# retinal-information-processing-lab/gaussian_processes

Measured on AMD Instinct MI355X. Metric: GP fits/sec (kernel+chol+solve+grad loglik) at N=8192 d=256, higher is better.
Workload: dtype f64; 1 GPU; N=8192 d=256 single cell f64, one M-step closure evaluation with 6 gradients (BASELINE configs[2], headline); N=8192, d=256, parallelism=independent units over 1 GPU(s), one process per GPU, no data-path collective

## Files before the change

gaussian_processes_amd/csrc/context.h:

```cpp
#pragma once
#include "kernels.h"
#include <vector>

struct gpfit_ctx {
  int device = 0;
  int np_cap = 0, dp_cap = 0, dfull_cap = 0;
  hipStream_t aux = nullptr;
  hipEvent_t ev_fork = nullptr, ev_join = nullptr;

  double *Kbuf = nullptr, *Cos = nullptr, *Lbuf = nullptr, *Libuf = nullptr, *Vbuf = nullptr, *LVbuf = nullptr,
         *LiVbuf = nullptr, *Tbuf = nullptr, *Zbuf = nullptr, *Wbuf = nullptr, *Abuf = nullptr, *Tmp = nullptr,
         *TmpV = nullptr;
  double *Xt = nullptr, *Xm = nullptr, *XCt = nullptr, *Cmat = nullptr, *Ybuf = nullptr, *Mpart = nullptr,
         *Mmat = nullptr, *Xt2 = nullptr, *XCt2 = nullptr, *XDt = nullptr, *XDt2 = nullptr, *dCpad = nullptr;
  double *Kvec = nullptr, *q = nullptr, *lam_m = nullptr, *lam_var = nullptr, *fvec = nullptr, *wl = nullptr,
         *yv = nullptr, *bv = nullptr, *tvec = nullptr , *mpad = nullptr, *rpad = nullptr,
         *q2 = nullptr, *dq1 = nullptr, *dq2 = nullptr, *hvec = nullptr;
  double *upart = nullptr, *vpart = nullptr, *sumA_part = nullptr, *frob_part = nullptr, *trmv_part = nullptr;
  double* rect_part = nullptr;
  void* sk_ws[2] = {nullptr, nullptr};
  hipStream_t side = nullptr;
  std::vector<hipEvent_t> side_ev;
  int side_ev_next = 0;
  double* scal = nullptr;
  double* scal_host = nullptr;
  int* pix = nullptr;
  int* pix_host = nullptr;
  int* info = nullptr;
  int* info_host = nullptr;
  std::vector<void*> allocs;
  int split_k_M = 32;

  int profile = 0;
  struct ProfRec { hipEvent_t a, b; double flops; int kind; };
  std::vector<ProfRec> prof;
  std::vector<hipEvent_t> ev_pool;
  double prof_out[16] = {0};
  hipEvent_t phase_ev[8] = {nullptr, nullptr, nullptr, nullptr, nullptr, nullptr, nullptr, nullptr};
  bool phase_valid = false;
  double last_enqueue_ms = 0.0;
  struct Pending { bool active = false; hipStream_t stream = nullptr; double A = 0, lambda0 = 0, sigma0 = 0;
                   int n = 0, np = 0, d = 0, want_grad = 0, elem_bytes = 8; hipEvent_t done = nullptr;
                   bool use_done = false; } pend;

  int cur_n = 0, cur_np = 0, cur_d = 0, cur_dp = 0;
  bool lv_valid = false;
  bool lv32_valid = false;
  int lv_n = 0;
  int lv_bytes = 0;
};

namespace gpfit {

struct DeviceGuard {
  int prev = -1;
  bool switched = false;
  explicit DeviceGuard(int device) {
    if (hipGetDevice(&prev) == hipSuccess && prev != device) switched = (hipSetDevice(device) == hipSuccess);
  }
  ~DeviceGuard() {
    if (switched) (void)hipSetDevice(prev);
  }
};
#define GP_CTX_ENTER(c, name)                                                                        \
  if ((c)->pend.active) {                                                                            \
    gpfit::set_error(name ": an asynchronous evaluation is pending on this context (collect it with " \
                          "gpfit_fit_eval_finish first)");                                           \
    return -3;                                                                                       \
  }                                                                                                  \
  gpfit::DeviceGuard _device_guard((c)->device)

void prof_begin(gpfit_ctx* c);
void prof_end(gpfit_ctx* c);
struct ProfScope {
  hipStream_t s; double flops; int kind; hipEvent_t a = nullptr;
  ProfScope(hipStream_t s, double flops, int kind);
  ~ProfScope();
};
template <typename R> double gemm_flops(const GemmArgsT<R>& g, int tile);

template <typename R>
struct CholBatchT {
  int nb = 0;
  R* A[GEMM_MAXB];
  R* L[GEMM_MAXB];
  R* Li[GEMM_MAXB];
  R* Tmp[GEMM_MAXB];
  int* info[GEMM_MAXB];
  int64_t ld = 0;
  void* sk_ws = nullptr;
  gpfit_ctx* ctx = nullptr;
  int side_min = 0;
};
template <typename R>
int potrf_lockstep(const CholBatchT<R>& B, int r0, int n, uint32_t need, hipStream_t s, uint32_t halves = 0);

}
```

gaussian_processes_amd/csrc/fit.hip:

```cpp
#include "context.h"
#include "gemm_core.h"
#include "gpfit_mi355x.h"

#include <algorithm>
#include <chrono>
#include <cmath>
#include <cstdlib>
#include <cstring>
#include <limits>

namespace gpfit {

static thread_local gpfit_ctx* g_prof = nullptr;
static thread_local void* g_main_sk_ws = nullptr;

static const int* walks() {
  static int w[7] = {3, 2, 1, 9, 9, 2, 2};
  static bool init = false;
  if (!init) {
    init = true;
    if (const char* e = getenv("GPFIT_WALKS")) {
      int v[7];
      if (sscanf(e, "%d,%d,%d,%d,%d,%d,%d", &v[0], &v[1], &v[2], &v[3], &v[4], &v[5], &v[6]) == 7)
        for (int i = 0; i < 7; ++i) w[i] = v[i];
// ... 147 lines not shown
                     int* sumsq_entries = nullptr) {
  if (epi_done) *epi_done = false;
  if (sumsq_entries) *sumsq_entries = 0;
  if (cnt <= 0) return 0;
  if (cnt > GEMM_MAXB) {
    set_error("gemm_list: more problems than a pointer batch holds");
    return -3;
  }
  GemmArgsT<R> g = gemm_args<R>(a_kmajor, b_kmajor, M, N, K, alpha, Ap[0], lda, Bp[0], ldb, beta, Cp[0], ldc, out_lower,
                                a_tri, b_tri, reverse, sk_ws);
  static const bool no_batch = getenv("GPFIT_NO_BATCH") != nullptr;
  if (cnt == 1 || gemm_pick_tile(g) == TILE || no_batch) {
    auto problem = [&](int i, bool fused) {
      g.A = Ap[i]; g.B = Bp[i]; g.C = Cp[i];
      g.epi = fused ? epi : 0; g.aux = (fused && auxp) ? auxp[i] : nullptr; g.sumsq = (fused && sumsqp) ? sumsqp[i] : nullptr;
    };
    GemmRoute routes[GEMM_MAXB];
    bool fused = epi != 0;
    for (int i = 0; i < cnt && fused; ++i) {
      problem(i, true);
      routes[i] = gemm_route(g);
      fused = routes[i].epi != 0;
    }
    for (int i = 0; i < cnt; ++i) {
      problem(i, fused);
      GP_TRY(fused ? run_gemm(s, g, routes[i]) : run_gemm(s, g));
    }
    if (epi_done) *epi_done = fused;
    if (fused && sumsq_entries) *sumsq_entries = routes[0].sumsq_entries;
    return 0;
  }
  g.nptr = cnt;
  g.batch = cnt;
  for (int i = 0; i < cnt; ++i) {
    g.Ap[i] = Ap[i]; g.Bp[i] = Bp[i]; g.Cp[i] = Cp[i];
    g.auxp[i] = auxp ? auxp[i] : nullptr; g.sumsqp[i] = sumsqp ? sumsqp[i] : nullptr;
  }
  g.epi = epi;
  GemmRoute r = gemm_route(g);
  if (epi && r.epi == 0) {
    g.epi = 0;
    r = gemm_route(g);
  }
  if (epi_done) *epi_done = g.epi != 0;
  if (sumsq_entries) *sumsq_entries = r.sumsq_entries;
  return run_gemm(s, g, r);
}

template <typename R>
static int bgemm(const CholBatchT<R>& B, hipStream_t s, uint32_t mask, int a_kmajor, int b_kmajor, int M, int N, int K,
                 double alpha, R* const* Ab, int64_t offA, R* const* Bb, int64_t offB, double beta, R* const* Cb,
                 int64_t offC, int out_lower, int a_tri, int b_tri, int reverse, void* sk_ws) {
  const R* Ap[GEMM_MAXB];
  const R* Bp[GEMM_MAXB];
  R* Cp[GEMM_MAXB];
  int cnt = 0;
  for (int b = 0; b < B.nb; ++b)
    if (mask & (1u << b)) {
      Ap[cnt] = Ab[b] + offA; Bp[cnt] = Bb[b] + offB; Cp[cnt] = Cb[b] + offC;
      ++cnt;
    }
  return gemm_list<R>(s, cnt, Ap, Bp, Cp, a_kmajor, b_kmajor, M, N, K, alpha, B.ld, B.ld, beta, B.ld, out_lower, a_tri,
                      b_tri, reverse, sk_ws);
}

template <typename R>
static GemmArgsT<R> batch_args(const CholBatchT<R>& B, uint32_t mask, int a_kmajor, int b_kmajor, int M, int N, int K, double alpha,
                               R* const* Ab, int64_t offA, R* const* Bb, int64_t offB, double beta, R* const* Cb, int64_t offC,
                               int out_lower, int a_tri, int b_tri, int reverse) {
  GemmArgsT<R> g = gemm_args<R>(a_kmajor, b_kmajor, M, N, K, alpha, (const R*)nullptr, B.ld, (const R*)nullptr, B.ld, beta,
                                (R*)nullptr, B.ld, out_lower, a_tri, b_tri, reverse, B.sk_ws);
  int cnt = 0;
  for (int b = 0; b < B.nb; ++b)
    if (mask & (1u << b)) {
      g.Ap[cnt] = Ab[b] + offA; g.Bp[cnt] = Bb[b] + offB; g.Cp[cnt] = Cb[b] + offC;
      ++cnt;
    }
  g.nptr = cnt;
  g.batch = cnt;
  if (cnt > 0) { g.A = g.Ap[0]; g.B = g.Bp[0]; g.C = g.Cp[0]; }
  return g;
}

template <typename R>
int potrf_lockstep(const CholBatchT<R>& B, int r0, int n, uint32_t need, hipStream_t s, uint32_t halves) {
  const int64_t ld = B.ld;
  const uint32_t all = (B.nb >= 32) ? 0xffffffffu : ((1u << B.nb) - 1u);
  auto off = [&](int r, int c) { return (int64_t)r * ld + c; };
  if (n == TILE) {
    ProfScope ps(s, 0.0, 1);
    LeafBatchT<R> bt{};
    bt.n = B.nb;
    for (int b = 0; b < B.nb; ++b) {
      bt.A[b] = B.A[b] + off(r0, r0); bt.L[b] = B.L[b] + off(r0, r0); bt.Li[b] = B.Li[b] + off(r0, r0);
      bt.info[b] = B.info[b];
    }
    bt.lda = bt.ldl = bt.ldi = ld;
    bt.info_base = r0;
    return launch_chol_leaf_batch(bt, s);
  }
  const int k = n / TILE;
  const int n1 = ((k + 1) / 2) * TILE, n2 = n - n1;
  const int r1 = r0 + n1;
  GP_TRY(potrf_lockstep<R>(B, r0, n1, all, s));
  GP_TRY(bgemm<R>(B, s, all, 0, 0, n2, n1, n1, 1.0, B.A, off(r1, r0), B.Li, off(r0, r0), 0.0, B.L, off(r1, r0), 0, 0, 2,
                  walks()[0], B.sk_ws));
  hipEvent_t joined = nullptr;
  if (need && B.ctx && B.side_min > 0 && n >= B.side_min && B.ctx->side) {
    gpfit_ctx* c = B.ctx;
    auto next_event = [&]() {
      if (c->side_ev_next == (int)c->side_ev.size()) {
        hipEvent_t e = nullptr;
        (void)hipEventCreateWithFlags(&e, hipEventDisableTiming);
        c->side_ev.push_back(e);
      }
      return c->side_ev[c->side_ev_next++];
    };
    hipEvent_t fork = next_event();
    joined = next_event();
    GP_HIP(hipEventRecord(fork, s));
    GP_HIP(hipStreamWaitEvent(c->side, fork, 0));
    GP_TRY(bgemm<R>(B, c->side, need, 0, 1, n2, n1, n1, 1.0, B.L, off(r1, r0), B.Li, off(r0, r0), 0.0, B.Tmp, off(r1, r0), 0, 0,
                    1, walks()[1], c->sk_ws[1]));
    GP_HIP(hipEventRecord(joined, c->side));
  }
  bool merged = false;
  if (need && !joined) {
    static const bool no_batch = getenv("GPFIT_NO_BATCH") != nullptr;
    const GemmArgsT<R> g2 = batch_args<R>(B, all, 0, 0, n2, n2, n1, -1.0, B.L, off(r1, r0), B.L, off(r1, r0), 1.0, B.A, off(r1, r1),
                                          1, 0, 0, 0);
    const GemmArgsT<R> g3 = batch_args<R>(B, need, 0, 1, n2, n1, n1, 1.0, B.L, off(r1, r0), B.Li, off(r0, r0), 0.0, B.Tmp,
                                          off(r1, r0), 0, 0, 1, walks()[1]);
    const GemmRoute pr = no_batch ? GemmRoute{} : gemm_pair_shape(g2, g3);
    if (!no_batch && pr.rc == 0) {
      if (gemm_log_eval() >= 0 && g_eval_count == gemm_log_eval())
        fprintf(stderr, "[gpfit gemm] pair: M %d N %d K %d lower 1 nb %d + M %d N %d K %d btri 1 nb %d tile %d flops %.6e\n", g2.M, g2.N,
                g2.K, g2.nptr, g3.M, g3.N, g3.K, g3.nptr, pr.tile, gemm_flops(g2, pr.tile) + gemm_flops(g3, pr.tile));
      ProfScope ps(s, g_prof ? gemm_flops(g2, pr.tile) + gemm_flops(g3, pr.tile) : 0.0, 3);
      GP_TRY(launch_gemm_pair(g2, g3, pr, s));
      merged = true;
    }
  }
  if (!merged)
    GP_TRY(bgemm<R>(B, s, all, 0, 0, n2, n2, n1, -1.0, B.L, off(r1, r0), B.L, off(r1, r0), 1.0, B.A, off(r1, r1), 1, 0, 0, 0,
                    B.sk_ws));
  GP_TRY(potrf_lockstep<R>(B, r1, n2, need | halves, s));
  if (need) {
    if (joined) GP_HIP(hipStreamWaitEvent(s, joined, 0));
    else if (!merged)
      GP_TRY(bgemm<R>(B, s, need, 0, 1, n2, n1, n1, 1.0, B.L, off(r1, r0), B.Li, off(r0, r0), 0.0, B.Tmp, off(r1, r0), 0, 0,
                      1, walks()[1], B.sk_ws));
    GP_TRY(bgemm<R>(B, s, need, 0, 1, n2, n1, n2, -1.0, B.Li, off(r1, r1), B.Tmp, off(r1, r0), 0.0, B.Li, off(r1, r0), 0, 1, 0,
                    walks()[2], B.sk_ws));
  }
  return 0;
}

template int potrf_lockstep<double>(const CholBatchT<double>&, int, int, uint32_t, hipStream_t, uint32_t);
template int potrf_lockstep<float>(const CholBatchT<float>&, int, int, uint32_t, hipStream_t, uint32_t);

template <typename R>
struct TwoSidedBufs {
  const R* Q; const R* Li; R* W; R* Z; R* H; int64_t ld; int min_split;
  void* sk_ws = nullptr;
};
template <typename R>
static int dual_update_list(hipStream_t s, int cnt, const R* const* Ap, const R* const* Bp, R* const* Hp, R* const* Zp, int M,
                            int N, int K, double alpha, int64_t ld, int b_tri, int walk, void* sk_ws) {
  bool fused = false;
  if (fused_epilogues() & 4) {
    GemmArgsT<R> g = gemm_args<R>(0, 1, M, N, K, alpha, Ap[0], ld, Bp[0], ld, 0.0, Hp[0], ld, 0, 0, b_tri, walk, sk_ws);
    g.epi = 4; g.aux = Zp[0];
    static const bool no_batch = getenv("GPFIT_NO_BATCH") != nullptr;
    if (cnt > 1 && gemm_pick_tile(g) != TILE && !no_batch) { g.nptr = cnt; g.batch = cnt; }
    fused = gemm_route(g).epi != 0;
  }
  if (fused) {
    bool done = false;
    GP_TRY(gemm_list<R>(s, cnt, Ap, Bp, Hp, 0, 1, M, N, K, alpha, ld, ld, 0.0, ld, 0, 0, b_tri, walk, sk_ws, 4, Zp, nullptr, &done));
    if (!done) {
      set_error("two_sided: the dual-update epilogue was announced but not carried");
      return -100;
    }
    return 0;
  }
  for (int i = 0; i < cnt; ++i)
    GP_HIP(hipMemcpy2DAsync(Hp[i], (size_t)ld * sizeof(R), Zp[i], (size_t)ld * sizeof(R), (size_t)N * sizeof(R), (size_t)M,
                            hipMemcpyDeviceToDevice, s));
  GP_TRY(gemm_list<R>(s, cnt, Ap, Bp, Hp, 0, 1, M, N, K, alpha, ld, ld, 1.0, ld, 0, 0, b_tri, walk, sk_ws));
  for (int i = 0; i < cnt; ++i) GP_TRY(launch_axpby_block<R>(Zp[i], ld, Hp[i], ld, M, N, 1.0, 1.0, s));
  return 0;
}

template <typename R>
static int two_sided_list(int cnt, const TwoSidedBufs<R>* b, const int* r0, int n, hipStream_t s) {
  if (cnt <= 0) return 0;
  const int64_t ld = b[0].ld;
  auto at = [&](const R* base, int r, int c) { return const_cast<R*>(base) + (int64_t)r * ld + c; };
  const R* Ap[GEMM_MAXB];
  const R* Bp[GEMM_MAXB];
  R* Cp[GEMM_MAXB];
  const int k = n / TILE;
  if (n < b[0].min_split || k < 2) {
    static const int wbase_walk = getenv("GPFIT_WBASE_WALK") ? atoi(getenv("GPFIT_WBASE_WALK")) : 0;
    for (int i = 0; i < cnt; ++i) { Ap[i] = at(b[i].Q, r0[i], r0[i]); Bp[i] = at(b[i].Li, r0[i], r0[i]); Cp[i] = at(b[i].Z, r0[i], r0[i]); }
    GP_TRY(gemm_list<R>(s, cnt, Ap, Bp, Cp, 1, 1, n, n, n, 1.0, ld, ld, 0.0, ld, 0, 0, 1, walks()[5], b[0].sk_ws));
    for (int i = 0; i < cnt; ++i) { Ap[i] = at(b[i].Li, r0[i], r0[i]); Bp[i] = at(b[i].Z, r0[i], r0[i]); Cp[i] = at(b[i].W, r0[i], r0[i]); }
    GP_TRY(gemm_list<R>(s, cnt, Ap, Bp, Cp, 1, 1, n, n, n, 0.5, ld, ld, 0.0, ld, 1, 2, 0, wbase_walk, b[0].sk_ws));
    return 0;
  }
  const int n1 = ((k + 1) / 2) * TILE, n2 = n - n1;
  auto diagonal_blocks = [&]() -> int {
    TwoSidedBufs<R> bb[GEMM_MAXB];
    int rr[GEMM_MAXB];
    if (n1 == n2 && 2 * cnt <= GEMM_MAXB) {
      for (int i = 0; i < cnt; ++i) {
        bb[2 * i] = b[i]; rr[2 * i] = r0[i];
        bb[2 * i + 1] = b[i]; rr[2 * i + 1] = r0[i] + n1;
      }
      return two_sided_list<R>(2 * cnt, bb, rr, n1, s);
    }
    for (int i = 0; i < cnt; ++i) rr[i] = r0[i] + n1;
    GP_TRY(two_sided_list<R>(cnt, b, r0, n1, s));
    return two_sided_list<R>(cnt, b, rr, n2, s);
  };
  for (int i = 0; i < cnt; ++i) {
    const int r1 = r0[i] + n1;
    Ap[i] = at(b[i].Q, r1, r1); Bp[i] = at(b[i].Li, r1, r0[i]); Cp[i] = at(b[i].Z, r1, r0[i]);
  }
// ... 288 lines not shown
}
static int projected_kl_products(gpfit_ctx* c, hipStream_t s, int nk, int nb) {
  double *Ki = c->Vbuf, *S2 = c->LVbuf, *S3 = c->LiVbuf, *S4 = c->TmpV;
  const int64_t lb = nb;
  GP_TRY(gemm<double>(s, 0, 1, nb, nb, nb, 1.0, Ki, lb, S2, lb, 0.0, S3, lb, 0, 0, 0));
  GP_TRY(launch_proj_trace(S3, lb, nk, c->scal + 5, s));
  return gemm<double>(s, 0, 1, nb, nb, nb, 1.0, S3, lb, Ki, lb, 0.0, S4, lb, 0, 0, 0);
}

static double sigma0_row_metric(const double* sc, double sigma0) { return sigma0 * (2.0 * sc[9] + 2.0 * sc[7]); }
static void grad_rows(const double* sc, double sigma0_row, double* g6) {
  g6[0] = sigma0_row;
  g6[1] = sc[13];
  g6[2] = sc[14];
  g6[3] = sc[11];
  g6[4] = sc[12];
  g6[5] = sc[10];
}
static int assemble_out(gpfit_ctx* c, double A, double lambda0, double sigma0_row, int pad, int d, int want_grad,
                        const char* err_K, const char* err_V, double* out_host) {
  const double* sc = c->scal_host;
  const double loglik = A * sc[0] + lambda0 * sc[1] - sc[2];
  const double trKinvV = sc[5] - (double)pad;
  const double logdetV = sc[40];
  const double KL = -0.5 * logdetV + 0.5 * sc[3] + 0.5 * sc[6] + 0.5 * trKinvV;
  out_host[0] = -(loglik - KL);
  out_host[1] = loglik;
  out_host[2] = KL;
  if (want_grad) grad_rows(sc, sigma0_row, out_host + 3);
  else
    for (int i = 0; i < 6; ++i) out_host[3 + i] = 0.0;
  out_host[9] = sc[3];
  out_host[10] = logdetV;
  out_host[11] = trKinvV;
  out_host[12] = sc[6];
  out_host[13] = (double)d;
  out_host[14] = (double)c->info_host[0];
  out_host[15] = (double)c->info_host[1];
  if (c->info_host[0] != 0) {
    set_error(err_K);
    return c->info_host[0];
  }
  if (c->info_host[1] != 0) {
    set_error(err_V);
    return c->info_host[1];
  }
  return 0;
}

template <typename R>
struct PostJoin {
  const R *Li, *L, *LV, *Cos, *bv, *q, *wl, *Xm, *Cmat;
  R *T, *W, *Z, *H, *A, *Y, *tvec, *Mpart, *Mmat;
};
template <typename R>
static PostJoin<R> post_join_args(gpfit_ctx* c) {
  auto RP = ws_as<R>;
  return PostJoin<R>{RP(c->Libuf), RP(c->Lbuf), RP(c->LVbuf), RP(c->Cos), RP(c->bv), RP(c->q), RP(c->wl), RP(c->Xm), RP(c->Cmat),
                     RP(c->Tbuf), RP(c->Wbuf), RP(c->Zbuf), RP(c->Tmp), RP(c->Abuf), RP(c->Ybuf), RP(c->tvec),
                     RP(c->Mpart), RP(c->Mmat)};
}
static int demote_for_mixed(gpfit_ctx* c, bool reuse_V, int np, int dp, bool blocks, hipStream_t s, PostJoin<float>* pf) {
  auto F = ws_as<float>;
  const int64_t nn = (int64_t)np * np;
  GP_TRY((launch_reduce_slices<double, float>(c->Libuf, nn, 1, F(c->Kbuf), nn, s)));
  if (blocks) {
    const int kt = np / TILE, n1 = ((kt + 1) / 2) * TILE;
    GP_TRY(launch_demote_block(c->Lbuf + (int64_t)n1 * np, np, F(c->Kbuf) + (int64_t)n1 * np, np, np - n1, n1, s));
  }
  if (!(reuse_V && c->lv32_valid)) GP_TRY((launch_reduce_slices<double, float>(c->LVbuf, nn, 1, F(c->Vbuf), nn, s)));
  c->lv32_valid = true;
  GP_TRY((launch_reduce_slices<double, float>(c->Cos, nn, 1, F(c->TmpV), nn, s)));
  GP_TRY((launch_reduce_slices<double, float>(c->bv, np, 1, F(c->q2), np, s)));
  GP_TRY((launch_reduce_slices<double, float>(c->q, np, 1, F(c->dq1), np, s)));
  GP_TRY((launch_reduce_slices<double, float>(c->wl, np, 1, F(c->dq2), np, s)));
  GP_TRY((launch_reduce_slices<double, float>(c->Xm, (int64_t)np * dp, 1, F(c->Xt2), (int64_t)np * dp, s)));
  GP_TRY((launch_reduce_slices<double, float>(c->Cmat, (int64_t)dp * dp, 1, F(c->dCpad), (int64_t)dp * dp, s)));
  *pf = PostJoin<float>{F(c->Kbuf), F(c->Kbuf), F(c->Vbuf), F(c->TmpV), F(c->q2), F(c->dq1), F(c->dq2), F(c->Xt2), F(c->dCpad),
                        F(c->Tbuf), F(c->Wbuf), F(c->Zbuf), F(c->Tmp), F(c->Abuf), F(c->Ybuf), F(c->tvec),
                        F(c->Mpart), F(c->Mmat)};
  return 0;
}

template <typename R>
static int t_in_blocks(int cnt, gpfit_ctx* const* cs, const PostJoin<R>* a, int np, hipStream_t s) {
  const int64_t ld = np;
  const R* Ap[GEMM_MAXB];
  const R* Bp[GEMM_MAXB];
  R* Cp[GEMM_MAXB];
  R* Tp[GEMM_MAXB];
  double* Sp[GEMM_MAXB];
  const int kt = np / TILE, n1 = ((kt + 1) / 2) * TILE, n2 = np - n1;
  int ent = 0;
  auto asks = [&](int M, int Nn, int K, int lower, int a_tri, int b_tri, int walk) {
    GemmArgsT<R> g1 = gemm_args<R>(0, 1, M, Nn, K, 1.0, a[0].Li, ld, a[0].LV, ld, 0.0, a[0].T, ld, lower, a_tri, b_tri, walk, cs[0]->sk_ws[0]);
    g1.epi = 2; g1.sumsq = cs[0]->frob_part;
    return (fused_epilogues() & 2) ? gemm_route(g1).sumsq_entries : 0;
  };
  const bool any_fused = asks(n1, n1, n1, 1, 1, 1, walks()[3]) > 0 || asks(n2, n2, n2, 1, 1, 1, walks()[3]) > 0 ||
                         asks(n2, n1, n2, 0, 1, 0, walks()[2]) > 0;
  auto diag_blocks = [&](int cb, const int* rb, int nblk) -> int {
    const int tb = nblk / TILE;
    int e = asks(nblk, nblk, nblk, 1, 1, 1, walks()[3]);
    const bool ask = e > 0;
    if (!ask) e = tb * (tb + 1) / 2;
    int m = 0;
    for (int i = 0; i < cnt; ++i)
      for (int j = 0; j < cb; ++j, ++m) {
        const int64_t o = (int64_t)rb[j] * ld + rb[j];
        Ap[m] = a[i].Li + o; Bp[m] = a[i].LV + o; Tp[m] = a[i].T + o; Sp[m] = cs[i]->frob_part + ent + j * e;
      }
    bool normed = false;
    GP_TRY(gemm_list<R>(s, m, Ap, Bp, Tp, 0, 1, nblk, nblk, nblk, 1.0, ld, ld, 0.0, ld, 1, 1, 1, walks()[3], cs[0]->sk_ws[0],
                        ask ? 2 : 0, nullptr, Sp, &normed));
    if (normed != ask) {
      set_error("post_join: the tile-norm epilogue of a diagonal block of T was announced but not carried");
      return -100;
    }
    if (!normed && any_fused)
      for (int q = 0; q < m; ++q) GP_TRY(launch_frob_tiles<R>(Tp[q], ld, nblk, nblk, 1, Sp[q], s));
    ent += cb * e;
    return 0;
  };
  const int r_both[2] = {0, n1};
  if (n2 == n1 && 2 * cnt <= GEMM_MAXB) GP_TRY(diag_blocks(2, r_both, n1));
  else {
    GP_TRY(diag_blocks(1, r_both, n1));
    GP_TRY(diag_blocks(1, r_both + 1, n2));
  }
  {
    const int64_t o21 = (int64_t)n1 * ld;
    for (int i = 0; i < cnt; ++i) {
      GP_HIP(hipMemcpy2DAsync(a[i].Z + o21, (size_t)ld * sizeof(R), a[i].LV + o21, (size_t)ld * sizeof(R), (size_t)n1 * sizeof(R),
                              (size_t)n2, hipMemcpyDeviceToDevice, s));
      Ap[i] = a[i].L + o21; Bp[i] = a[i].T; Cp[i] = a[i].Z + o21;
    }
    GP_TRY(gemm_list<R>(s, cnt, Ap, Bp, Cp, 0, 1, n2, n1, n1, -1.0, ld, ld, 1.0, ld, 0, 0, 1, walks()[1], cs[0]->sk_ws[0]));
    int e = asks(n2, n1, n2, 0, 1, 0, walks()[2]);
    const bool ask = e > 0;
    if (!ask) e = (n2 / TILE) * (n1 / TILE);
    for (int i = 0; i < cnt; ++i) {
      Ap[i] = a[i].Li + o21 + n1; Bp[i] = a[i].Z + o21; Tp[i] = a[i].T + o21; Sp[i] = cs[i]->frob_part + ent;
    }
    bool normed = false;
    GP_TRY(gemm_list<R>(s, cnt, Ap, Bp, Tp, 0, 1, n2, n1, n2, 1.0, ld, ld, 0.0, ld, 0, 1, 0, walks()[2], cs[0]->sk_ws[0],
                        ask ? 2 : 0, nullptr, Sp, &normed));
    if (normed != ask) {
      set_error("post_join: the tile-norm epilogue of T21 was announced but not carried");
      return -100;
    }
    if (!normed && any_fused)
      for (int i = 0; i < cnt; ++i) GP_TRY(launch_frob_tiles<R>(Tp[i], ld, n2, n1, 0, Sp[i], s));
    ent += e;
  }
  for (int i = 0; i < cnt; ++i) {
    if (any_fused) GP_TRY(launch_frob_finish(cs[i]->frob_part, ent, cs[i]->scal + 5, s));
    else GP_TRY(launch_frob_lower(a[i].T, ld, np, cs[i]->scal + 5, cs[i]->frob_part, s));
  }
  return 0;
}

template <typename R, typename PhaseFn>
static int post_join_list(int cnt, gpfit_ctx* const* cs, const PostJoin<R>* a, const Theta* th, int n, int np, const int* d,
                          const int* dp, int n_rows, int n_cols, int want_grad, bool blocks, hipStream_t s, PhaseFn&& phase) {
  const int64_t ld = np;
  const R* Ap[GEMM_MAXB];
  const R* Bp[GEMM_MAXB];
  R* Cp[GEMM_MAXB];
  R* Sp2[GEMM_MAXB];
  double* Sp[GEMM_MAXB];
  if (cnt <= 0 || cnt > GEMM_MAXB) return cnt == 0 ? 0 : -3;
  if (!blocks) {
    for (int i = 0; i < cnt; ++i) { Ap[i] = a[i].Li; Bp[i] = a[i].LV; Cp[i] = a[i].T; Sp[i] = cs[i]->frob_part; }
    bool normed = false;
    int norm_entries = 0;
    GP_TRY(gemm_list<R>(s, cnt, Ap, Bp, Cp, 0, 1, np, np, np, 1.0, ld, ld, 0.0, ld, 1, 1, 1, walks()[3], cs[0]->sk_ws[0],
                        (fused_epilogues() & 2) ? 2 : 0, nullptr, Sp, &normed, &norm_entries));
    for (int i = 0; i < cnt; ++i) {
      if (normed) GP_TRY(launch_frob_finish(cs[i]->frob_part, norm_entries, cs[i]->scal + 5, s));
      else GP_TRY(launch_frob_lower(a[i].T, ld, np, cs[i]->scal + 5, cs[i]->frob_part, s));
    }
  } else {
    GP_TRY(t_in_blocks<R>(cnt, cs, a, np, s));
  }
  phase(4, s);
  if (!want_grad) return 0;
  {
    for (int i = 0; i < cnt; ++i) { Ap[i] = a[i].T; Bp[i] = a[i].T; Cp[i] = a[i].W; }
    bool mirrored = false;
    GP_TRY(gemm_list<R>(s, cnt, Ap, Bp, Cp, 0, 0, np, np, np, -1.0, ld, ld, 0.0, ld, 1, 1, 2, walks()[4], cs[0]->sk_ws[0],
                        (fused_epilogues() & 1) ? 1 : 0, nullptr, nullptr, &mirrored));
    for (int i = 0; i < cnt; ++i) {
      GP_TRY(launch_add_diag(a[i].W, ld, np, 1.0, s));
      if (!mirrored) GP_TRY(launch_symmetrize(a[i].W, ld, np, s));
    }
  }
  phase(5, s);
  {
    static const int ts_min = getenv("GPFIT_TS_MIN") ? atoi(getenv("GPFIT_TS_MIN")) : 4096;
    TwoSidedBufs<R> tb[GEMM_MAXB];
    const R* Lf[GEMM_MAXB];
    for (int i = 0; i < cnt; ++i) {
      tb[i] = TwoSidedBufs<R>{a[i].W, a[i].Li, a[i].T, a[i].Z, a[i].H, ld, ts_min > 0 ? ts_min : (1 << 30)};
      tb[i].sk_ws = cs[0]->sk_ws[0];
      Lf[i] = a[i].L;
    }
    if (blocks) GP_TRY(two_sided_top<R>(cnt, tb, Lf, np, s));
    else {
      int r0[GEMM_MAXB];
      for (int i = 0; i < cnt; ++i) r0[i] = 0;
      GP_TRY(two_sided_list<R>(cnt, tb, r0, np, s));
    }
  }
  phase(6, s);
  for (int i = 0; i < cnt; ++i)
    GP_TRY(adjoint_pass<R>(cs[i], s, a[i].T, a[i].Cos, a[i].bv, a[i].q, a[i].wl, n, np, a[i].A, a[i].tvec));
  {
    bool same_dp = true;
    for (int i = 1; i < cnt; ++i) same_dp = same_dp && dp[i] == dp[0];
    for (int i = 0; i < cnt; ++i) { Ap[i] = a[i].A; Bp[i] = a[i].Xm; Cp[i] = a[i].Y; Sp2[i] = a[i].Z; }
    if (same_dp) GP_TRY(lambda_t_x_list<R>(s, cnt, Ap, Bp, Cp, Sp2, np, dp[0]));
    else
      for (int i = 0; i < cnt; ++i) GP_TRY(lambda_t_x_list<R>(s, 1, Ap + i, Bp + i, Cp + i, Sp2 + i, np, dp[i]));
  }
  for (int i = 0; i < cnt; ++i) {
    gpfit_ctx* c = cs[i];
    GP_TRY(launch_rowscale_add(a[i].Y, dp[i], a[i].Xm, dp[i], a[i].tvec, np, dp[i], s, 0.5));
    GP_TRY(xty<R>(c, s, a[i].Xm, a[i].Y, np, dp[i], a[i].Mmat, true, true));
    GP_TRY(launch_metric_contract(th[i], c->pix, d[i], n_rows, n_cols, a[i].Cmat, dp[i], a[i].Mmat, dp[i], c->scal + 10, c->upart,
                                  c->info + 3, s));
  }
  return 0;
}

static void set_pending(gpfit_ctx* c, hipStream_t s, double A, double lambda0, double sigma0, int n, int np, int d,
                        int want_grad, int elem_bytes, bool use_done) {
  c->pend.active = true; c->pend.stream = s; c->pend.A = A; c->pend.lambda0 = lambda0; c->pend.sigma0 = sigma0;
  c->pend.n = n; c->pend.np = np; c->pend.d = d; c->pend.want_grad = want_grad; c->pend.elem_bytes = elem_bytes;
  c->pend.use_done = use_done;
}

int fit_eval_finish(gpfit_ctx* c, double* out_host);

template <typename R>
static int fit_eval_impl(gpfit_ctx* c, void* stream, const double* theta, const double* lower, const double* upper,
                         int n_rows, int n_cols, const R* X, int64_t ldx, int64_t N, const R* r, const R* m,
                         const R* V, int64_t ldv, double logA, double lambda0, int want_grad, double* out_host,
                         R* lam_m_out, R* lam_var_out, R* f_out) {
  auto RP = ws_as<R>;
  if (!c || !theta || !X || !r || !m || !V || !out_host || N <= 0) {
    set_error("gpfit_fit_eval: bad argument");
    return -3;
  }
  GP_CTX_ENTER(c, "gpfit_fit_eval");
  hipStream_t s = (hipStream_t)stream;
  const int n = (int)N, np = (int)round_up(N, TILE);
  Admitted ad;
  GP_TRY(admit(c, "gpfit_fit_eval", "the context", theta, lower, upper, n_rows, n_cols, np, out_host, &ad));
  const int d = ad.d, dp = ad.dp;
  const Theta th = ad.th;
  const double A = std::exp(logA);
  const int64_t ld = np;
  const bool blocks = top_in_blocks(np, sizeof(R));
  c->cur_n = n; c->cur_np = np; c->cur_d = d; c->cur_dp = dp;

  ++g_eval_count;
  const auto t_host0 = std::chrono::steady_clock::now();
  auto phase = [&](int i, hipStream_t st) {
    if (c->profile != 2) return;
    if (!c->phase_ev[i]) (void)hipEventCreate(&c->phase_ev[i]);
    (void)hipEventRecord(c->phase_ev[i], st);
  };
  c->phase_valid = false;
  phase(0, s);
  g_main_sk_ws = c->sk_ws[0];
  prof_begin(c);
  struct ProfGuard { gpfit_ctx* c; ~ProfGuard() { prof_end(c); } } prof_guard{c};
  GP_HIP(hipMemsetAsync(c->info, 0, 4 * sizeof(int), s));
  GP_HIP(hipMemcpyAsync(c->pix, c->pix_host, (size_t)d * sizeof(int), hipMemcpyHostToDevice, s));
  GP_HIP(hipMemsetAsync(RP(c->mpad), 0, (size_t)np * sizeof(R), s));
  GP_HIP(hipMemcpyAsync(RP(c->mpad), m, (size_t)n * sizeof(R), hipMemcpyDeviceToDevice, s));

  const bool reuse_V = (want_grad & 2) && c->lv_valid && c->lv_n == n && c->lv_bytes == (int)sizeof(R);
  const bool async_call = (want_grad & 4) != 0;
  const bool mixed_grad = (want_grad & 8) != 0 && sizeof(R) == 8 && (want_grad & 1);
  want_grad &= 1;
  static const int side_min_env = getenv("GPFIT_SIDE_MIN") ? atoi(getenv("GPFIT_SIDE_MIN")) : 1024;
  const int side_min = async_call ? 0 : side_min_env;
  if (!async_call) GP_TRY(ensure_side_stream(c));
  c->side_ev_next = 0;
  if (!reuse_V) {
    c->lv_valid = false; c->lv32_valid = false;
    GP_HIP(hipEventRecord(c->ev_fork, s));
    GP_HIP(hipStreamWaitEvent(c->aux, c->ev_fork, 0));
    GP_TRY(launch_pack_lower(V, ldv, n, RP(c->Vbuf), ld, np, c->aux));
    GP_HIP(hipEventRecord(c->ev_join, c->aux));
  }

  GP_TRY(build_kernel<R>(c, s, th, d, dp, n_rows, n_cols, X, ldx, n, np, 0));
  GP_TRY(launch_moments(RP(c->Kvec), RP(c->q), RP(c->Cos), ld, V, ldv, m, r, n, A, lambda0, RP(c->lam_m), RP(c->lam_var), RP(c->fvec),
                        RP(c->wl), c->scal, c->sumA_part, c->info + 2, s));
  phase(1, s);
  {
    CholBatchT<R> cb;
    cb.nb = reuse_V ? 1 : 2;
    cb.A[0] = RP(c->Kbuf); cb.L[0] = RP(c->Lbuf); cb.Li[0] = RP(c->Libuf); cb.Tmp[0] = RP(c->Tmp); cb.info[0] = c->info + 0;
    cb.A[1] = RP(c->Vbuf); cb.L[1] = RP(c->LVbuf); cb.Li[1] = RP(c->LiVbuf); cb.Tmp[1] = RP(c->TmpV); cb.info[1] = c->info + 1;
    cb.ld = ld; cb.sk_ws = c->sk_ws[0]; cb.ctx = c; cb.side_min = side_min;
    if (!reuse_V) GP_HIP(hipStreamWaitEvent(s, c->ev_join, 0));
    if (blocks) GP_TRY(potrf_lockstep<R>(cb, 0, np, 0u, s, 1u));
    else GP_TRY(potrf_lockstep<R>(cb, 0, np, 1u, s));
    if (!reuse_V) GP_TRY(launch_logdet(RP(c->LVbuf), ld, n, c->scal + 40, s));
    phase(3, s);
  }
  GP_TRY(launch_logdet(RP(c->Lbuf), ld, n, c->scal + 3, s));
  GP_TRY(solve_mean<R>(c, np, blocks, s));

  phase(2, s);
  if (mixed_grad) {
    PostJoin<float> pf;
    GP_TRY(demote_for_mixed(c, reuse_V, np, dp, blocks, s, &pf));
    GP_TRY(post_join_list<float>(1, &c, &pf, &th, n, np, &d, &dp, n_rows, n_cols, want_grad, blocks, s, phase));
  } else {
    const PostJoin<R> pj = post_join_args<R>(c);
    GP_TRY(post_join_list<R>(1, &c, &pj, &th, n, np, &d, &dp, n_rows, n_cols, want_grad, blocks, s, phase));
  }

  if (lam_m_out) GP_HIP(hipMemcpyAsync(lam_m_out, RP(c->lam_m), (size_t)n * sizeof(R), hipMemcpyDeviceToDevice, s));
  if (lam_var_out) GP_HIP(hipMemcpyAsync(lam_var_out, RP(c->lam_var), (size_t)n * sizeof(R), hipMemcpyDeviceToDevice, s));
  if (f_out) GP_HIP(hipMemcpyAsync(f_out, RP(c->fvec), (size_t)n * sizeof(R), hipMemcpyDeviceToDevice, s));
  GP_HIP(hipMemcpyAsync(c->scal_host, c->scal, 64 * sizeof(double), hipMemcpyDeviceToHost, s));
  GP_HIP(hipMemcpyAsync(c->info_host, c->info, 4 * sizeof(int), hipMemcpyDeviceToHost, s));
  phase(7, s);
  c->phase_valid = (c->profile == 2 && want_grad && !reuse_V);
  c->last_enqueue_ms = std::chrono::duration<double, std::milli>(std::chrono::steady_clock::now() - t_host0).count();
  set_pending(c, s, A, lambda0, th.sigma0, n, np, d, want_grad, (int)sizeof(R), false);
  if (async_call) return 0;
  return fit_eval_finish(c, out_host);
}

template <typename R>
static int fit_eval_batch_impl(gpfit_ctx* const* cs, int nu, void* stream, const double* theta6, const double* lower,
                               const double* upper, int n_rows, int n_cols, const R* const* X, int64_t ldx, int64_t N,
                               const R* const* r, const R* const* m, const R* const* V, int64_t ldv, const double* logA,
                               const double* lambda0, int want_grad, double* out_host, int* rc_out) {
  auto RP = ws_as<R>;
  if (!cs || nu <= 0 || 2 * nu > GEMM_MAXB || !theta6 || !X || !r || !m || !V || !logA || !lambda0 || !out_host || !rc_out ||
      N <= 0) {
    set_error("gpfit_fit_eval_batch: bad argument (1 .. 16 units per call)");
    return -3;
  }
  for (int u = 0; u < nu; ++u) {
    if (!cs[u] || !X[u] || !r[u] || !m[u] || !V[u]) {
      set_error("gpfit_fit_eval_batch: null context or operand");
      return -3;
    }
    if (cs[u]->device != cs[0]->device) {
      set_error("gpfit_fit_eval_batch: the contexts of one call must live on one device");
      return -3;
    }
    for (int v = 0; v < u; ++v)
      if (cs[v] == cs[u]) {
        set_error("gpfit_fit_eval_batch: every unit needs a context of its own");
        return -3;
      }
    if (cs[u]->pend.active) {
      set_error("gpfit_fit_eval_batch: an asynchronous evaluation is pending on one of the contexts");
      return -3;
    }
  }
  DeviceGuard device_guard(cs[0]->device);
  hipStream_t s = (hipStream_t)stream;
  const int n = (int)N, np = (int)round_up(N, TILE);
  const int64_t ld = np;
  const bool mixed_grad = (want_grad & 8) != 0 && sizeof(R) == 8 && (want_grad & 1);
  const bool want_reuse = (want_grad & 2) != 0;
  const bool blocks = top_in_blocks(np, sizeof(R));
  want_grad &= 1;
  const auto t_host0 = std::chrono::steady_clock::now();

  struct Unit { gpfit_ctx* c; int u, d, dp; Theta th; double A; bool reuse_V; };
  Unit un[GEMM_MAXB];
  int na = 0;
  for (int u = 0; u < nu; ++u) {
    gpfit_ctx* c = cs[u];
    Admitted ad;
    const int rc = admit(c, "gpfit_fit_eval_batch", "a context's", theta6 + 6 * u, lower, upper, n_rows, n_cols, np,
                         out_host + 16 * u, &ad);
    rc_out[u] = rc == -2 ? -2 : 0;
    if (rc == -2) continue;
    if (rc != 0) return rc;
    Unit& q = un[na++];
    q.c = c; q.u = u; q.d = ad.d; q.dp = ad.dp; q.th = ad.th; q.A = std::exp(logA[u]);
    q.reuse_V = want_reuse && c->lv_valid && c->lv_n == n && c->lv_bytes == (int)sizeof(R);
    c->cur_n = n; c->cur_np = np; c->cur_d = q.d; c->cur_dp = q.dp;
    c->phase_valid = false;
    c->side_ev_next = 0;
  }
  if (na == 0) return 0;
  gpfit_ctx* c0 = un[0].c;
  static const bool batch_times = getenv("GPFIT_BATCH_TIMES") != nullptr;
  hipEvent_t tev[4] = {nullptr, nullptr, nullptr, nullptr};
  if (batch_times) {
    for (auto& e : tev) (void)hipEventCreate(&e);
    (void)hipEventRecord(tev[0], s);
  }
  {
    GroupPrepT<R> gp{};
// ... 529 lines not shown
```

Baseline: 36.65 fits/s.

## Overlap early T-block GEMMs on side stream with trailing Cholesky recursion

Adds a hook at the top level of the recursive lockstep Cholesky. Once the leading half is factored, it forks the T11 diagonal block and the S off-diagonal update onto the side stream, where they overlap with factoring the trailing half. The remaining T22/T21 blocks and the norm run after a join. This aims to fill idle compute during the serial trailing factorization, at the cost of extra stream events, contention for the GPU between the two streams, and a half-occupancy setting on the S GEMM.

```diff
diff --git a/gaussian_processes_amd/csrc/context.h b/gaussian_processes_amd/csrc/context.h
--- a/gaussian_processes_amd/csrc/context.h
+++ b/gaussian_processes_amd/csrc/context.h
@@ -91,6 +91,9 @@
   void* sk_ws = nullptr;
   gpfit_ctx* ctx = nullptr;
   int side_min = 0;
+  int top_n = 0;
+  int (*top_hook)(void* arg, hipStream_t s) = nullptr;
+  void* top_arg = nullptr;
 };
 template <typename R>
 int potrf_lockstep(const CholBatchT<R>& B, int r0, int n, uint32_t need, hipStream_t s, uint32_t halves = 0);
diff --git a/gaussian_processes_amd/csrc/fit.hip b/gaussian_processes_amd/csrc/fit.hip
--- a/gaussian_processes_amd/csrc/fit.hip
+++ b/gaussian_processes_amd/csrc/fit.hip
@@ -253,6 +253,15 @@
   return g;
 }
 
+static hipEvent_t side_event(gpfit_ctx* c) {
+  if (c->side_ev_next == (int)c->side_ev.size()) {
+    hipEvent_t e = nullptr;
+    (void)hipEventCreateWithFlags(&e, hipEventDisableTiming);
+    c->side_ev.push_back(e);
+  }
+  return c->side_ev[c->side_ev_next++];
+}
+
 template <typename R>
 int potrf_lockstep(const CholBatchT<R>& B, int r0, int n, uint32_t need, hipStream_t s, uint32_t halves) {
   const int64_t ld = B.ld;
@@ -279,16 +288,8 @@
   hipEvent_t joined = nullptr;
   if (need && B.ctx && B.side_min > 0 && n >= B.side_min && B.ctx->side) {
     gpfit_ctx* c = B.ctx;
-    auto next_event = [&]() {
-      if (c->side_ev_next == (int)c->side_ev.size()) {
-        hipEvent_t e = nullptr;
-        (void)hipEventCreateWithFlags(&e, hipEventDisableTiming);
-        c->side_ev.push_back(e);
-      }
-      return c->side_ev[c->side_ev_next++];
-    };
-    hipEvent_t fork = next_event();
-    joined = next_event();
+    hipEvent_t fork = side_event(c);
+    joined = side_event(c);
     GP_HIP(hipEventRecord(fork, s));
     GP_HIP(hipStreamWaitEvent(c->side, fork, 0));
     GP_TRY(bgemm<R>(B, c->side, need, 0, 1, n2, n1, n1, 1.0, B.L, off(r1, r0), B.Li, off(r0, r0), 0.0, B.Tmp, off(r1, r0), 0, 0,
@@ -315,7 +316,14 @@
   if (!merged)
     GP_TRY(bgemm<R>(B, s, all, 0, 0, n2, n2, n1, -1.0, B.L, off(r1, r0), B.L, off(r1, r0), 1.0, B.A, off(r1, r1), 1, 0, 0, 0,
                     B.sk_ws));
-  GP_TRY(potrf_lockstep<R>(B, r1, n2, need | halves, s));
+  if (B.top_hook && r0 == 0 && n == B.top_n) {
+    GP_TRY(B.top_hook(B.top_arg, s));
+    CholBatchT<R> B2 = B;
+    B2.top_hook = nullptr; B2.side_min = 0;
+    GP_TRY(potrf_lockstep<R>(B2, r1, n2, need | halves, s));
+  } else {
+    GP_TRY(potrf_lockstep<R>(B, r1, n2, need | halves, s));
+  }
   if (need) {
     if (joined) GP_HIP(hipStreamWaitEvent(s, joined, 0));
     else if (!merged)
@@ -770,8 +778,10 @@
   return 0;
 }
 
-template <typename R>
-static int t_in_blocks(int cnt, gpfit_ctx* const* cs, const PostJoin<R>* a, int np, hipStream_t s) {
+enum : int { T_11 = 1, T_S = 2, T_EARLY = 3, T_LATE = 4, T_ALL = 7 };
+template <typename R>
+static int t_in_blocks(int cnt, gpfit_ctx* const* cs, const PostJoin<R>* a, int np, hipStream_t s, int stages = T_ALL,
+                       void* sk_ws = nullptr, bool s_half_occ = false) {
   const int64_t ld = np;
   const R* Ap[GEMM_MAXB];
   const R* Bp[GEMM_MAXB];
@@ -779,7 +789,7 @@
   R* Tp[GEMM_MAXB];
   double* Sp[GEMM_MAXB];
   const int kt = np / TILE, n1 = ((kt + 1) / 2) * TILE, n2 = np - n1;
-  int ent = 0;
+  void* sk = sk_ws ? sk_ws : cs[0]->sk_ws[0];
   auto asks = [&](int M, int Nn, int K, int lower, int a_tri, int b_tri, int walk) {
     GemmArgsT<R> g1 = gemm_args<R>(0, 1, M, Nn, K, 1.0, a[0].Li, ld, a[0].LV, ld, 0.0, a[0].T, ld, lower, a_tri, b_tri, walk, cs[0]->sk_ws[0]);
     g1.epi = 2; g1.sumsq = cs[0]->frob_part;
@@ -787,11 +797,13 @@
   };
   const bool any_fused = asks(n1, n1, n1, 1, 1, 1, walks()[3]) > 0 || asks(n2, n2, n2, 1, 1, 1, walks()[3]) > 0 ||
                          asks(n2, n1, n2, 0, 1, 0, walks()[2]) > 0;
-  auto diag_blocks = [&](int cb, const int* rb, int nblk) -> int {
-    const int tb = nblk / TILE;
-    int e = asks(nblk, nblk, nblk, 1, 1, 1, walks()[3]);
-    const bool ask = e > 0;
-    if (!ask) e = tb * (tb + 1) / 2;
+  auto diag_entries = [&](int nblk) {
+    const int tb = nblk / TILE, e = asks(nblk, nblk, nblk, 1, 1, 1, walks()[3]);
+    return e > 0 ? e : tb * (tb + 1) / 2;
+  };
+  auto diag_blocks = [&](int cb, const int* rb, int nblk, int ent) -> int {
+    const bool ask = asks(nblk, nblk, nblk, 1, 1, 1, walks()[3]) > 0;
+    const int e = diag_entries(nblk);
     int m = 0;
     for (int i = 0; i < cnt; ++i)
       for (int j = 0; j < cb; ++j, ++m) {
@@ -799,7 +811,7 @@
         Ap[m] = a[i].Li + o; Bp[m] = a[i].LV + o; Tp[m] = a[i].T + o; Sp[m] = cs[i]->frob_part + ent + j * e;
       }
     bool normed = false;
-    GP_TRY(gemm_list<R>(s, m, Ap, Bp, Tp, 0, 1, nblk, nblk, nblk, 1.0, ld, ld, 0.0, ld, 1, 1, 1, walks()[3], cs[0]->sk_ws[0],
+    GP_TRY(gemm_list<R>(s, m, Ap, Bp, Tp, 0, 1, nblk, nblk, nblk, 1.0, ld, ld, 0.0, ld, 1, 1, 1, walks()[3], sk,
                         ask ? 2 : 0, nullptr, Sp, &normed));
     if (normed != ask) {
       set_error("post_join: the tile-norm epilogue of a diagonal block of T was announced but not carried");
@@ -807,31 +819,33 @@
     }
     if (!normed && any_fused)
       for (int q = 0; q < m; ++q) GP_TRY(launch_frob_tiles<R>(Tp[q], ld, nblk, nblk, 1, Sp[q], s));
-    ent += cb * e;
     return 0;
   };
   const int r_both[2] = {0, n1};
-  if (n2 == n1 && 2 * cnt <= GEMM_MAXB) GP_TRY(diag_blocks(2, r_both, n1));
-  else {
-    GP_TRY(diag_blocks(1, r_both, n1));
-    GP_TRY(diag_blocks(1, r_both + 1, n2));
-  }
-  {
-    const int64_t o21 = (int64_t)n1 * ld;
+  const int64_t o21 = (int64_t)n1 * ld;
+  const int ent22 = diag_entries(n1), ent21 = ent22 + diag_entries(n2);
+  auto s_block = [&]() -> int {
     for (int i = 0; i < cnt; ++i) {
       GP_HIP(hipMemcpy2DAsync(a[i].Z + o21, (size_t)ld * sizeof(R), a[i].LV + o21, (size_t)ld * sizeof(R), (size_t)n1 * sizeof(R),
                               (size_t)n2, hipMemcpyDeviceToDevice, s));
       Ap[i] = a[i].L + o21; Bp[i] = a[i].T; Cp[i] = a[i].Z + o21;
     }
-    GP_TRY(gemm_list<R>(s, cnt, Ap, Bp, Cp, 0, 1, n2, n1, n1, -1.0, ld, ld, 1.0, ld, 0, 0, 1, walks()[1], cs[0]->sk_ws[0]));
+    if (s_half_occ && cnt == 1) {
+      GemmArgsT<R> g = gemm_args<R>(0, 1, n2, n1, n1, -1.0, Ap[0], ld, Bp[0], ld, 1.0, Cp[0], ld, 0, 0, 1, walks()[1], sk);
+      g.half_occ = 1;
+      return run_gemm(s, g);
+    }
+    return gemm_list<R>(s, cnt, Ap, Bp, Cp, 0, 1, n2, n1, n1, -1.0, ld, ld, 1.0, ld, 0, 0, 1, walks()[1], sk);
+  };
+  auto t21_and_norm = [&]() -> int {
     int e = asks(n2, n1, n2, 0, 1, 0, walks()[2]);
     const bool ask = e > 0;
     if (!ask) e = (n2 / TILE) * (n1 / TILE);
     for (int i = 0; i < cnt; ++i) {
-      Ap[i] = a[i].Li + o21 + n1; Bp[i] = a[i].Z + o21; Tp[i] = a[i].T + o21; Sp[i] = cs[i]->frob_part + ent;
+      Ap[i] = a[i].Li + o21 + n1; Bp[i] = a[i].Z + o21; Tp[i] = a[i].T + o21; Sp[i] = cs[i]->frob_part + ent21;
     }
     bool normed = false;
-    GP_TRY(gemm_list<R>(s, cnt, Ap, Bp, Tp, 0, 1, n2, n1, n2, 1.0, ld, ld, 0.0, ld, 0, 1, 0, walks()[2], cs[0]->sk_ws[0],
+    GP_TRY(gemm_list<R>(s, cnt, Ap, Bp, Tp, 0, 1, n2, n1, n2, 1.0, ld, ld, 0.0, ld, 0, 1, 0, walks()[2], sk,
                         ask ? 2 : 0, nullptr, Sp, &normed));
     if (normed != ask) {
       set_error("post_join: the tile-norm epilogue of T21 was announced but not carried");
@@ -839,18 +853,34 @@
     }
     if (!normed && any_fused)
       for (int i = 0; i < cnt; ++i) GP_TRY(launch_frob_tiles<R>(Tp[i], ld, n2, n1, 0, Sp[i], s));
-    ent += e;
-  }
-  for (int i = 0; i < cnt; ++i) {
-    if (any_fused) GP_TRY(launch_frob_finish(cs[i]->frob_part, ent, cs[i]->scal + 5, s));
-    else GP_TRY(launch_frob_lower(a[i].T, ld, np, cs[i]->scal + 5, cs[i]->frob_part, s));
+    for (int i = 0; i < cnt; ++i) {
+      if (any_fused) GP_TRY(launch_frob_finish(cs[i]->frob_part, ent21 + e, cs[i]->scal + 5, s));
+      else GP_TRY(launch_frob_lower(a[i].T, ld, np, cs[i]->scal + 5, cs[i]->frob_part, s));
+    }
+    return 0;
+  };
+  if (stages == T_ALL) {
+    if (n2 == n1 && 2 * cnt <= GEMM_MAXB) GP_TRY(diag_blocks(2, r_both, n1, 0));
+    else {
+      GP_TRY(diag_blocks(1, r_both, n1, 0));
+      GP_TRY(diag_blocks(1, r_both + 1, n2, ent22));
+    }
+    GP_TRY(s_block());
+    return t21_and_norm();
+  }
+  if (stages & T_11) GP_TRY(diag_blocks(1, r_both, n1, 0));
+  if (stages & T_S) GP_TRY(s_block());
+  if (stages & T_LATE) {
+    GP_TRY(diag_blocks(1, r_both + 1, n2, ent22));
+    GP_TRY(t21_and_norm());
   }
   return 0;
 }
 
 template <typename R, typename PhaseFn>
 static int post_join_list(int cnt, gpfit_ctx* const* cs, const PostJoin<R>* a, const Theta* th, int n, int np, const int* d,
-                          const int* dp, int n_rows, int n_cols, int want_grad, bool blocks, hipStream_t s, PhaseFn&& phase) {
+                          const int* dp, int n_rows, int n_cols, int want_grad, bool blocks, hipStream_t s, PhaseFn&& phase,
+                          int t_stages = T_ALL) {
   const int64_t ld = np;
   const R* Ap[GEMM_MAXB];
   const R* Bp[GEMM_MAXB];
@@ -869,7 +899,7 @@
       else GP_TRY(launch_frob_lower(a[i].T, ld, np, cs[i]->scal + 5, cs[i]->frob_part, s));
     }
   } else {
-    GP_TRY(t_in_blocks<R>(cnt, cs, a, np, s));
+    GP_TRY(t_in_blocks<R>(cnt, cs, a, np, s, t_stages));
   }
   phase(4, s);
   if (!want_grad) return 0;
@@ -927,6 +957,42 @@
   c->pend.n = n; c->pend.np = np; c->pend.d = d; c->pend.want_grad = want_grad; c->pend.elem_bytes = elem_bytes;
   c->pend.use_done = use_done;
 }
+
+static int early_t_mode() {
+  static const int v = getenv("GPFIT_EARLY_T") ? atoi(getenv("GPFIT_EARLY_T")) : 1;
+  return v;
+}
+template <typename R>
+struct EarlyT {
+  gpfit_ctx* c;
+  PostJoin<R> pj;
+  int np;
+  hipEvent_t done = nullptr;
+  bool forked = false, joined = false;
+  static int fork(void* arg, hipStream_t s) {
+    EarlyT* e = static_cast<EarlyT*>(arg);
+    gpfit_ctx* c = e->c;
+    const bool t11_on_main = early_t_mode() == 2;
+    if (t11_on_main) GP_TRY(t_in_blocks<R>(1, &c, &e->pj, e->np, s, T_11, c->sk_ws[0]));
+    hipEvent_t ev = side_event(c);
+    e->done = side_event(c);
+    GP_HIP(hipEventRecord(ev, s));
+    GP_HIP(hipStreamWaitEvent(c->side, ev, 0));
+    e->forked = true;
+    GP_TRY(t_in_blocks<R>(1, &c, &e->pj, e->np, c->side, t11_on_main ? T_S : T_EARLY, c->sk_ws[1], true));
+    GP_HIP(hipEventRecord(e->done, c->side));
+    return 0;
+  }
+  int join(hipStream_t s) {
+    if (!forked || joined) return 0;
+    GP_HIP(hipStreamWaitEvent(s, done, 0));
+    joined = true;
+    return 0;
+  }
+  ~EarlyT() {
+    if (forked && !joined) (void)hipStreamSynchronize(c->side);
+  }
+};
 
 int fit_eval_finish(gpfit_ctx* c, double* out_host);
 
@@ -977,6 +1043,8 @@
   const int side_min = async_call ? 0 : side_min_env;
   if (!async_call) GP_TRY(ensure_side_stream(c));
   c->side_ev_next = 0;
+  const bool early_t = early_t_mode() > 0 && blocks && !async_call && !mixed_grad && !reuse_V && c->side != nullptr;
+  EarlyT<R> early{c, post_join_args<R>(c), np};
   if (!reuse_V) {
     c->lv_valid = false; c->lv32_valid = false;
     GP_HIP(hipEventRecord(c->ev_fork, s));
@@ -995,6 +1063,7 @@
     cb.A[0] = RP(c->Kbuf); cb.L[0] = RP(c->Lbuf); cb.Li[0] = RP(c->Libuf); cb.Tmp[0] = RP(c->Tmp); cb.info[0] = c->info + 0;
     cb.A[1] = RP(c->Vbuf); cb.L[1] = RP(c->LVbuf); cb.Li[1] = RP(c->LiVbuf); cb.Tmp[1] = RP(c->TmpV); cb.info[1] = c->info + 1;
     cb.ld = ld; cb.sk_ws = c->sk_ws[0]; cb.ctx = c; cb.side_min = side_min;
+    if (early_t) { cb.top_n = np; cb.top_hook = &EarlyT<R>::fork; cb.top_arg = &early; }
     if (!reuse_V) GP_HIP(hipStreamWaitEvent(s, c->ev_join, 0));
     if (blocks) GP_TRY(potrf_lockstep<R>(cb, 0, np, 0u, s, 1u));
     else GP_TRY(potrf_lockstep<R>(cb, 0, np, 1u, s));
@@ -1010,8 +1079,9 @@
     GP_TRY(demote_for_mixed(c, reuse_V, np, dp, blocks, s, &pf));
     GP_TRY(post_join_list<float>(1, &c, &pf, &th, n, np, &d, &dp, n_rows, n_cols, want_grad, blocks, s, phase));
   } else {
-    const PostJoin<R> pj = post_join_args<R>(c);
-    GP_TRY(post_join_list<R>(1, &c, &pj, &th, n, np, &d, &dp, n_rows, n_cols, want_grad, blocks, s, phase));
+    GP_TRY(early.join(s));
+    GP_TRY(post_join_list<R>(1, &c, &early.pj, &th, n, np, &d, &dp, n_rows, n_cols, want_grad, blocks, s, phase,
+                             early.forked ? T_LATE : T_ALL));
   }
 
   if (lam_m_out) GP_HIP(hipMemcpyAsync(lam_m_out, RP(c->lam_m), (size_t)n * sizeof(R), hipMemcpyDeviceToDevice, s));
```

Measured after the change: 37.05 fits/s (median of 6 runs). +1.1%, better.
